# 3SAILab/two_stage_object_detection

Measured on AMD Instinct MI355X. Metric: images/sec Faster R-CNN ResNet-50 @800x1333, higher is better.
Workload: dtype f32 storage/accumulate; conv products as bf16x3 (3 exact bf16 pieces per operand, 6 bf16 MFMAs per product) in 0 of 43 conv layers, as fp16x2 (2 fp16 pieces of 2^e x per operand, 3 fp16 MFMAs per product; e follows the tensor's abs-max per forward: range words) in 43, f32 MFMA in the rest; 1 GPU; Full Faster R-CNN resnet50 inference forward, batch=1 per GPU, 3x800x1333, 80+1 classes, 3000->300 proposals; global_batch=1, parallelism=dp1, hip_graph=True, autotuned_tiles=True, steps_in_flight=4, tiles_tuned_on=this rank

## Files before the change

### two_stage_object_detection_amd/csrc/roi_pool.hip

```cpp
#include "tsod_internal.h"
#include <float.h>
#include <math.h>

namespace {

__device__ __forceinline__ float4 max4(float4 m, const float4 v) {
    if (v.x > m.x) m.x = v.x;
    if (v.y > m.y) m.y = v.y;
    if (v.z > m.z) m.z = v.z;
    if (v.w > m.w) m.w = v.w;
    return m;
}

__device__ __forceinline__ float4 bin_max(const float *__restrict__ fmap, int Wf, int pitch, int c4, int hs, int he,
                                          int ws, int we) {
    if (he <= hs || we <= ws) return make_float4(0.f, 0.f, 0.f, 0.f);
    float4 m = make_float4(-FLT_MAX, -FLT_MAX, -FLT_MAX, -FLT_MAX);
    for (int h = hs; h < he; ++h) {
        const float *rowp = fmap + ((long)h * Wf) * pitch + 4 * c4;
        for (int w = ws; w < we; ++w) m = max4(m, *reinterpret_cast<const float4 *>(rowp + (long)w * pitch));
    }
    return m;
}

__global__ void __launch_bounds__(256)
roi_pool_kernel(const float *__restrict__ feat, int B, int Hf, int Wf, int C, int pitch,
                const float *__restrict__ rois5, float scale, int PH, int PW, float *__restrict__ out) {
    const int k = blockIdx.x;
    const float *r = rois5 + 5l * k;
    const tsod_pool_geom g = tsod_roi_pool_geom(r[0], r[1], r[2], r[3], r[4], scale);
    if (g.b < 0 || g.b >= B) return;
    const float bin_h = (float)g.rh / (float)PH;
    const float bin_w = (float)g.rw / (float)PW;
    const float *fmap = feat + (long)g.b * Hf * Wf * pitch;
    const int bins = PH * PW;
    for (int c4 = threadIdx.x; c4 < (C >> 2); c4 += blockDim.x) {
        for (int ph = 0; ph < PH; ++ph) {
            int hs, he;
            tsod_bin_range(ph, bin_h, g.sh, Hf, hs, he);
            for (int pw = 0; pw < PW; ++pw) {
                int ws, we;
                tsod_bin_range(pw, bin_w, g.sw, Wf, ws, we);
                const float4 m = bin_max(fmap, Wf, pitch, c4, hs, he, ws, we);
                float *o = out + ((long)k * C + 4 * c4) * bins + ph * PW + pw;
                o[0] = m.x; o[bins] = m.y; o[2 * bins] = m.z; o[3 * bins] = m.w;
            }
        }
    }
}

constexpr int kQuads = 32;

__global__ void __launch_bounds__(256)
roi_pool_avg_kernel(const float *__restrict__ feat, int B, int Hf, int Wf, int C, int pitch,
                    const float *__restrict__ rois, const int *__restrict__ roi_indices, int R,
                    float img_h, float img_w, float scale, int PH, int PW, float *__restrict__ out, int out_pitch, int roi_in_y) {
    __shared__ float4 rowsum[8][kQuads];
    const int k = roi_in_y ? blockIdx.y : blockIdx.x;
    const float4 rr = reinterpret_cast<const float4 *>(rois)[k];
    const float4 fm = tsod_roi_to_map(rr, img_h, img_w, Hf, Wf);
    const tsod_pool_geom g = tsod_roi_pool_geom((float)roi_indices[k / R], fm.x, fm.y, fm.z, fm.w, scale);
    if (g.b < 0 || g.b >= B) return;
    const float bin_h = (float)g.rh / (float)PH;
    const float bin_w = (float)g.rw / (float)PW;
    const float *fmap = feat + (long)g.b * Hf * Wf * pitch;
    const float nb = (float)(PH * PW);
    const int q = threadIdx.x % kQuads, slot = threadIdx.x / kQuads;
    const int c4 = (roi_in_y ? blockIdx.x : blockIdx.y) * kQuads + q;
    const bool live = c4 < (C >> 2);
    float4 total = make_float4(0.f, 0.f, 0.f, 0.f);
    for (int ph0 = 0; ph0 < PH; ph0 += 8) {
        const int ph = ph0 + slot;
        float4 acc = make_float4(0.f, 0.f, 0.f, 0.f);
        if (live && ph < PH) {
            int hs, he;
            tsod_bin_range(ph, bin_h, g.sh, Hf, hs, he);
            int kept_x = -1;
            float4 kept = make_float4(-FLT_MAX, -FLT_MAX, -FLT_MAX, -FLT_MAX);
            for (int pw = 0; pw < PW; ++pw) {
                int ws, we;
                tsod_bin_range(pw, bin_w, g.sw, Wf, ws, we);
                float4 m = make_float4(0.f, 0.f, 0.f, 0.f);
                if (he > hs && we > ws) {
                    m = make_float4(-FLT_MAX, -FLT_MAX, -FLT_MAX, -FLT_MAX);
                    for (int w = ws; w < we; ++w) {
                        float4 col = kept;
                        if (w != kept_x) {
                            col = make_float4(-FLT_MAX, -FLT_MAX, -FLT_MAX, -FLT_MAX);
                            const float *colp = fmap + ((long)hs * Wf + w) * pitch + 4 * c4;
                            for (int h = hs; h < he; ++h, colp += (long)Wf * pitch) col = max4(col, *reinterpret_cast<const float4 *>(colp));
                        }
                        m = max4(m, col);
                        if (w == we - 1) { kept = col; kept_x = w; }
                    }
                }
                acc.x += m.x; acc.y += m.y; acc.z += m.z; acc.w += m.w;
            }
        }
        rowsum[slot][q] = acc;
        __syncthreads();
        if (slot == 0) {
            const int rows = min(8, PH - ph0);
            for (int r = 0; r < rows; ++r) {
                const float4 v = rowsum[r][q];
                total.x += v.x; total.y += v.y; total.z += v.z; total.w += v.w;
            }
        }
        __syncthreads();
    }
    if (slot == 0 && live)
        *reinterpret_cast<float4 *>(out + (long)k * out_pitch + 4 * c4) =
            make_float4(total.x / nb, total.y / nb, total.z / nb, total.w / nb);
}

__device__ __forceinline__ float4 align_bin_sum(const float *__restrict__ fmap, int Hf, int Wf, int pitch, int c4,
                                                const tsod_align_geom &g, int ph, int pw) {
    float4 acc = make_float4(0.f, 0.f, 0.f, 0.f);
    for (int iy = 0; iy < g.grid_h; ++iy) {
        const float yy = TSOD_ALIGN_SAMPLE(g.start_h, g.bin_h, g.grid_h, ph, iy);
        for (int ix = 0; ix < g.grid_w; ++ix) {
            const float xx = TSOD_ALIGN_SAMPLE(g.start_w, g.bin_w, g.grid_w, pw, ix);
            TSOD_ALIGN_BILINEAR_OR_CONTINUE(yy, xx, Hf, Wf);
            const float hy = 1.f - ly, hx = 1.f - lx;
            const float w1 = hy * hx, w2 = hy * lx, w3 = ly * hx, w4 = ly * lx;
            const float4 v1 = *reinterpret_cast<const float4 *>(fmap + ((long)y_low * Wf + x_low) * pitch + 4 * c4);
            const float4 v2 = *reinterpret_cast<const float4 *>(fmap + ((long)y_low * Wf + x_high) * pitch + 4 * c4);
            const float4 v3 = *reinterpret_cast<const float4 *>(fmap + ((long)y_high * Wf + x_low) * pitch + 4 * c4);
            const float4 v4 = *reinterpret_cast<const float4 *>(fmap + ((long)y_high * Wf + x_high) * pitch + 4 * c4);
            acc.x += w1 * v1.x + w2 * v2.x + w3 * v3.x + w4 * v4.x;
            acc.y += w1 * v1.y + w2 * v2.y + w3 * v3.y + w4 * v4.y;
            acc.z += w1 * v1.z + w2 * v2.z + w3 * v3.z + w4 * v4.z;
            acc.w += w1 * v1.w + w2 * v2.w + w3 * v3.w + w4 * v4.w;
        }
    }
    return acc;
}

__global__ void __launch_bounds__(256)
roi_align_kernel(const float *__restrict__ feat, int B, int Hf, int Wf, int C, int pitch, const float *__restrict__ rois5,
                 float scale, int PH, int PW, int sampling_ratio, int aligned, float *__restrict__ out) {
    const int k = blockIdx.x;
    const float *r = rois5 + 5l * k;
    const tsod_align_geom g = tsod_roi_align_geom(r[0], r[1], r[2], r[3], r[4], scale, PH, PW, sampling_ratio, aligned);
    if (g.b < 0 || g.b >= B) return;
    const float *fmap = feat + (long)g.b * Hf * Wf * pitch;
    const int bins = PH * PW, quads = C >> 2;
    for (int t = threadIdx.x; t < quads * bins; t += blockDim.x) {
        const int c4 = t % quads, bin = t / quads;
        const float4 sum = align_bin_sum(fmap, Hf, Wf, pitch, c4, g, bin / PW, bin % PW);
        float *o = out + ((long)k * C + 4 * c4) * bins + bin;
        o[0] = sum.x / g.count; o[bins] = sum.y / g.count; o[2 * bins] = sum.z / g.count; o[3 * bins] = sum.w / g.count;
    }
}

__global__ void __launch_bounds__(256)
roi_align_avg_kernel(const float *__restrict__ feat, int B, int Hf, int Wf, int C, int pitch, const float *__restrict__ rois,
                     const int *__restrict__ roi_indices, int R, float img_h, float img_w, float scale, int PH, int PW,
                     int sampling_ratio, int aligned, float *__restrict__ out, int out_pitch, int roi_in_y) {
    __shared__ float4 rowsum[8][kQuads];
    const int k = roi_in_y ? blockIdx.y : blockIdx.x;
    const float4 rr = reinterpret_cast<const float4 *>(rois)[k];
    const float4 fm = tsod_roi_to_map(rr, img_h, img_w, Hf, Wf);
    const tsod_align_geom g = tsod_roi_align_geom((float)roi_indices[k / R], fm.x, fm.y, fm.z, fm.w, scale, PH, PW, sampling_ratio,
                                                  aligned);
    if (g.b < 0 || g.b >= B) return;
    const float *fmap = feat + (long)g.b * Hf * Wf * pitch;
    const float nb = (float)(PH * PW);
    const int q = threadIdx.x % kQuads, slot = threadIdx.x / kQuads;
    const int c4 = (roi_in_y ? blockIdx.x : blockIdx.y) * kQuads + q;
    const bool live = c4 < (C >> 2);
    float4 total = make_float4(0.f, 0.f, 0.f, 0.f);
    for (int ph0 = 0; ph0 < PH; ph0 += 8) {
        const int ph = ph0 + slot;
        float4 acc = make_float4(0.f, 0.f, 0.f, 0.f);
        if (live && ph < PH) {
            for (int pw = 0; pw < PW; ++pw) {
                const float4 s4 = align_bin_sum(fmap, Hf, Wf, pitch, c4, g, ph, pw);
                acc.x += s4.x / g.count; acc.y += s4.y / g.count; acc.z += s4.z / g.count; acc.w += s4.w / g.count;
            }
        }
        rowsum[slot][q] = acc;
        __syncthreads();
        if (slot == 0) {
            const int rows = min(8, PH - ph0);
            for (int r = 0; r < rows; ++r) {
                const float4 v = rowsum[r][q];
                total.x += v.x; total.y += v.y; total.z += v.z; total.w += v.w;
            }
        }
        __syncthreads();
    }
    if (slot == 0 && live)
        *reinterpret_cast<float4 *>(out + (long)k * out_pitch + 4 * c4) =
            make_float4(total.x / nb, total.y / nb, total.z / nb, total.w / nb);
}

}

extern "C" int tsod_roi_align_f32(const float *feat, int32_t B, int32_t Hf, int32_t Wf, int32_t C, int32_t feat_pitch,
                                  const float *rois5, int32_t K, float spatial_scale, int32_t PH, int32_t PW,
                                  int32_t sampling_ratio, int32_t aligned, float *out, tsod_stream_t stream) {
    TSOD_REQUIRE(feat && rois5 && out, TSOD_ERR_INVALID_ARG);
    TSOD_REQUIRE(B > 0 && Hf > 0 && Wf > 0 && C > 0 && K > 0 && PH > 0 && PW > 0 && sampling_ratio >= 0, TSOD_ERR_INVALID_ARG);
    TSOD_REQUIRE((C & 3) == 0 && (feat_pitch & 3) == 0 && feat_pitch >= C && tsod_aligned16(feat), TSOD_ERR_ALIGNMENT);
    hipLaunchKernelGGL(roi_align_kernel, dim3(K), dim3(256), 0, tsod_stream(stream), feat, B, Hf, Wf, C, feat_pitch, rois5,
                       spatial_scale, PH, PW, sampling_ratio, aligned ? 1 : 0, out);
    return tsod_launch_status();
}

extern "C" int tsod_roi_align_avg_f32(const float *feat, int32_t B, int32_t Hf, int32_t Wf, int32_t C, int32_t feat_pitch,
                                      const float *rois, const int32_t *roi_indices, int32_t R, float img_h, float img_w,
                                      float spatial_scale, int32_t PH, int32_t PW, int32_t sampling_ratio, int32_t aligned,
                                      float *out, int32_t out_pitch, tsod_stream_t stream) {
    TSOD_REQUIRE(feat && rois && roi_indices && out, TSOD_ERR_INVALID_ARG);
    TSOD_REQUIRE(B > 0 && Hf > 0 && Wf > 0 && C > 0 && R > 0 && PH > 0 && PW > 0 && PH <= 64 && sampling_ratio >= 0,
                 TSOD_ERR_INVALID_ARG);
    TSOD_REQUIRE(img_h > 0.f && img_w > 0.f, TSOD_ERR_INVALID_ARG);
    TSOD_REQUIRE((C & 3) == 0 && (feat_pitch & 3) == 0 && feat_pitch >= C && (out_pitch & 3) == 0 && out_pitch >= C,
                 TSOD_ERR_ALIGNMENT);
    TSOD_REQUIRE(tsod_aligned16(feat) && tsod_aligned16(rois) && tsod_aligned16(out), TSOD_ERR_ALIGNMENT);
    const int quads = C / 4;
    const int groups = (quads + kQuads - 1) / kQuads, roi_in_y = (long)B * R <= 65535 ? 1 : 0;
    hipLaunchKernelGGL(roi_align_avg_kernel, roi_in_y ? dim3(groups, B * R) : dim3(B * R, groups), dim3(256), 0, tsod_stream(stream),
                       feat, B, Hf, Wf, C, feat_pitch, rois, roi_indices, R, img_h, img_w, spatial_scale, PH, PW,
                       sampling_ratio, aligned ? 1 : 0, out, out_pitch, roi_in_y);
    return tsod_launch_status();
}

extern "C" int tsod_roi_pool_f32(const float *feat, int32_t B, int32_t Hf, int32_t Wf, int32_t C, int32_t feat_pitch,
                                 const float *rois5, int32_t K, float spatial_scale, int32_t PH, int32_t PW,
                                 float *out, tsod_stream_t stream) {
    TSOD_REQUIRE(feat && rois5 && out, TSOD_ERR_INVALID_ARG);
    TSOD_REQUIRE(B > 0 && Hf > 0 && Wf > 0 && C > 0 && K > 0 && PH > 0 && PW > 0, TSOD_ERR_INVALID_ARG);
    TSOD_REQUIRE((C & 3) == 0 && (feat_pitch & 3) == 0 && feat_pitch >= C && tsod_aligned16(feat), TSOD_ERR_ALIGNMENT);
    hipLaunchKernelGGL(roi_pool_kernel, dim3(K), dim3(256), 0, tsod_stream(stream), feat, B, Hf, Wf, C, feat_pitch,
                       rois5, spatial_scale, PH, PW, out);
    return tsod_launch_status();
}

extern "C" int tsod_roi_pool_avg_f32(const float *feat, int32_t B, int32_t Hf, int32_t Wf, int32_t C,
                                     int32_t feat_pitch, const float *rois, const int32_t *roi_indices, int32_t R,
                                     float img_h, float img_w, float spatial_scale, int32_t PH, int32_t PW, float *out,
                                     int32_t out_pitch, tsod_stream_t stream) {
    TSOD_REQUIRE(feat && rois && roi_indices && out, TSOD_ERR_INVALID_ARG);
    TSOD_REQUIRE(B > 0 && Hf > 0 && Wf > 0 && C > 0 && R > 0 && PH > 0 && PW > 0, TSOD_ERR_INVALID_ARG);
    TSOD_REQUIRE(img_h > 0.f && img_w > 0.f, TSOD_ERR_INVALID_ARG);
    TSOD_REQUIRE((C & 3) == 0 && (feat_pitch & 3) == 0 && feat_pitch >= C && (out_pitch & 3) == 0 && out_pitch >= C,
                 TSOD_ERR_ALIGNMENT);
    TSOD_REQUIRE(tsod_aligned16(feat) && tsod_aligned16(rois) && tsod_aligned16(out), TSOD_ERR_ALIGNMENT);
    const int quads = C / 4;
    const int groups = (quads + kQuads - 1) / kQuads, roi_in_y = (long)B * R <= 65535 ? 1 : 0;
    hipLaunchKernelGGL(roi_pool_avg_kernel, roi_in_y ? dim3(groups, B * R) : dim3(B * R, groups), dim3(256), 0, tsod_stream(stream), feat, B, Hf,
                       Wf, C, feat_pitch, rois, roi_indices, R, img_h, img_w, spatial_scale, PH, PW, out, out_pitch, roi_in_y);
    return tsod_launch_status();
}
```

Measured before the change: 1208 images/s.

## Restructure avg ROI pool to wave-uniform rows with readlane bin ranges

The avg ROI-pool kernel now maps 64 channel quads to each wavefront so that each wave handles one pooled row, and makes the row range scalar via readfirstlane. Column bin ranges are computed once per lane and broadcast with readlane instead of being recomputed serially. The row loop is unrolled by four with 32-bit offsets. The block size now scales with PH, up to 512 threads. The aim is to cut divergent per-thread bin arithmetic and raise memory-level parallelism. The cost is larger blocks and a new limit that Wf*pitch must fit in 32 bits.

```diff
diff --git a/two_stage_object_detection_amd/csrc/roi_pool.hip b/two_stage_object_detection_amd/csrc/roi_pool.hip
--- a/two_stage_object_detection_amd/csrc/roi_pool.hip
+++ b/two_stage_object_detection_amd/csrc/roi_pool.hip
@@ -49,13 +49,16 @@
     }
 }
 
+constexpr int kRowQuads = 64;
 constexpr int kQuads = 32;
 
-__global__ void __launch_bounds__(256)
+__device__ __forceinline__ float4 ld4(const float *p) { return *reinterpret_cast<const float4 *>(p); }
+
+__global__ void __launch_bounds__(512)
 roi_pool_avg_kernel(const float *__restrict__ feat, int B, int Hf, int Wf, int C, int pitch,
                     const float *__restrict__ rois, const int *__restrict__ roi_indices, int R,
                     float img_h, float img_w, float scale, int PH, int PW, float *__restrict__ out, int out_pitch, int roi_in_y) {
-    __shared__ float4 rowsum[8][kQuads];
+    __shared__ float4 rowsum[8][kRowQuads];
     const int k = roi_in_y ? blockIdx.y : blockIdx.x;
     const float4 rr = reinterpret_cast<const float4 *>(rois)[k];
     const float4 fm = tsod_roi_to_map(rr, img_h, img_w, Hf, Wf);
@@ -63,46 +66,71 @@
     if (g.b < 0 || g.b >= B) return;
     const float bin_h = (float)g.rh / (float)PH;
     const float bin_w = (float)g.rw / (float)PW;
-    const float *fmap = feat + (long)g.b * Hf * Wf * pitch;
     const float nb = (float)(PH * PW);
-    const int q = threadIdx.x % kQuads, slot = threadIdx.x / kQuads;
-    const int c4 = (roi_in_y ? blockIdx.x : blockIdx.y) * kQuads + q;
+    const int lane = threadIdx.x % kRowQuads;
+    const int slot = __builtin_amdgcn_readfirstlane(threadIdx.x / kRowQuads);
+    const int nw = blockDim.x / kRowQuads;
+    const int c0 = (roi_in_y ? blockIdx.x : blockIdx.y) * kRowQuads, c4 = c0 + lane;
     const bool live = c4 < (C >> 2);
+    const float *gmap = feat + (long)g.b * Hf * Wf * pitch + 4 * c0;
+    const unsigned lq = live ? 4u * lane : 0u;
+    const long rs = (long)Wf * pitch;
     float4 total = make_float4(0.f, 0.f, 0.f, 0.f);
-    for (int ph0 = 0; ph0 < PH; ph0 += 8) {
+    for (int ph0 = 0; ph0 < PH; ph0 += nw) {
         const int ph = ph0 + slot;
         float4 acc = make_float4(0.f, 0.f, 0.f, 0.f);
-        if (live && ph < PH) {
-            int hs, he;
-            tsod_bin_range(ph, bin_h, g.sh, Hf, hs, he);
+        int hs = 0, he = 0;
+        if (ph < PH) tsod_bin_range(ph, bin_h, g.sh, Hf, hs, he);
+        hs = __builtin_amdgcn_readfirstlane(hs);
+        he = __builtin_amdgcn_readfirstlane(he);
+        if (he > hs) {
+            const float *prow = gmap + hs * rs;
             int kept_x = -1;
             float4 kept = make_float4(-FLT_MAX, -FLT_MAX, -FLT_MAX, -FLT_MAX);
-            for (int pw = 0; pw < PW; ++pw) {
-                int ws, we;
-                tsod_bin_range(pw, bin_w, g.sw, Wf, ws, we);
-                float4 m = make_float4(0.f, 0.f, 0.f, 0.f);
-                if (he > hs && we > ws) {
-                    m = make_float4(-FLT_MAX, -FLT_MAX, -FLT_MAX, -FLT_MAX);
-                    for (int w = ws; w < we; ++w) {
-                        float4 col = kept;
-                        if (w != kept_x) {
-                            col = make_float4(-FLT_MAX, -FLT_MAX, -FLT_MAX, -FLT_MAX);
-                            const float *colp = fmap + ((long)hs * Wf + w) * pitch + 4 * c4;
-                            for (int h = hs; h < he; ++h, colp += (long)Wf * pitch) col = max4(col, *reinterpret_cast<const float4 *>(colp));
+            for (int pw0 = 0; pw0 < PW; pw0 += 64) {
+                int ws_l, we_l;
+                tsod_bin_range(pw0 + (int)(threadIdx.x % 64), bin_w, g.sw, Wf, ws_l, we_l);
+                const int pw1 = min(pw0 + 64, PW);
+                for (int pw = pw0; pw < pw1; ++pw) {
+                    const int ws = __builtin_amdgcn_readlane(ws_l, pw - pw0), we = __builtin_amdgcn_readlane(we_l, pw - pw0);
+                    float4 m = make_float4(0.f, 0.f, 0.f, 0.f);
+                    if (we > ws) {
+                        m = make_float4(-FLT_MAX, -FLT_MAX, -FLT_MAX, -FLT_MAX);
+                        for (int w = ws; w < we; ++w) {
+                            float4 col = kept;
+                            if (w != kept_x) {
+                                col = make_float4(-FLT_MAX, -FLT_MAX, -FLT_MAX, -FLT_MAX);
+                                const float *colp = prow + w * pitch;
+                                int n = he - hs;
+                                for (; n >= 4; n -= 4, colp += 4 * rs) {
+                                    const float4 a = ld4(colp + lq), b = ld4(colp + rs + lq), c = ld4(colp + 2 * rs + lq),
+                                                 d = ld4(colp + 3 * rs + lq);
+                                    col = max4(max4(max4(max4(col, a), b), c), d);
+                                }
+                                if (n == 3) {
+                                    const float4 a = ld4(colp + lq), b = ld4(colp + rs + lq), c = ld4(colp + 2 * rs + lq);
+                                    col = max4(max4(max4(col, a), b), c);
+                                } else if (n == 2) {
+                                    const float4 a = ld4(colp + lq), b = ld4(colp + rs + lq);
+                                    col = max4(max4(col, a), b);
+                                } else if (n == 1) {
+                                    col = max4(col, ld4(colp + lq));
+                                }
+                            }
+                            m = max4(m, col);
+                            if (w == we - 1) { kept = col; kept_x = w; }
                         }
-                        m = max4(m, col);
-                        if (w == we - 1) { kept = col; kept_x = w; }
                     }
+                    acc.x += m.x; acc.y += m.y; acc.z += m.z; acc.w += m.w;
                 }
-                acc.x += m.x; acc.y += m.y; acc.z += m.z; acc.w += m.w;
-            }
-        }
-        rowsum[slot][q] = acc;
+            }
+        }
+        rowsum[slot][lane] = acc;
         __syncthreads();
         if (slot == 0) {
-            const int rows = min(8, PH - ph0);
+            const int rows = min(nw, PH - ph0);
             for (int r = 0; r < rows; ++r) {
-                const float4 v = rowsum[r][q];
+                const float4 v = rowsum[r][lane];
                 total.x += v.x; total.y += v.y; total.z += v.z; total.w += v.w;
             }
         }
@@ -248,9 +276,10 @@
     TSOD_REQUIRE((C & 3) == 0 && (feat_pitch & 3) == 0 && feat_pitch >= C && (out_pitch & 3) == 0 && out_pitch >= C,
                  TSOD_ERR_ALIGNMENT);
     TSOD_REQUIRE(tsod_aligned16(feat) && tsod_aligned16(rois) && tsod_aligned16(out), TSOD_ERR_ALIGNMENT);
+    TSOD_REQUIRE((long)Wf * feat_pitch <= 0x7fffffffl, TSOD_ERR_INVALID_ARG);
     const int quads = C / 4;
-    const int groups = (quads + kQuads - 1) / kQuads, roi_in_y = (long)B * R <= 65535 ? 1 : 0;
-    hipLaunchKernelGGL(roi_pool_avg_kernel, roi_in_y ? dim3(groups, B * R) : dim3(B * R, groups), dim3(256), 0, tsod_stream(stream), feat, B, Hf,
+    const int groups = (quads + kRowQuads - 1) / kRowQuads, roi_in_y = (long)B * R <= 65535 ? 1 : 0;
+    hipLaunchKernelGGL(roi_pool_avg_kernel, roi_in_y ? dim3(groups, B * R) : dim3(B * R, groups), dim3(kRowQuads * (PH < 8 ? PH : 8)), 0, tsod_stream(stream), feat, B, Hf,
                        Wf, C, feat_pitch, rois, roi_indices, R, img_h, img_w, spatial_scale, PH, PW, out, out_pitch, roi_in_y);
     return tsod_launch_status();
 }
```

New measurement: 1211 images/s, median of 3. Within noise of the previous version (+0.3%).
